# raywan-110/AdaQP

Hardware: NVIDIA H100
Metric: epochs_per_sec (higher is better)
Workload: dtype f32

## Files before the change

### adaqp_b200/_lib.py

```python
from __future__ import annotations

import ctypes as C
import os

import numpy as np

HERE = os.path.dirname(os.path.abspath(__file__))
LIB_PATH = os.path.join(HERE, "libadaqp_b200.so")

c_void_p = C.c_void_p
i64 = C.c_int64
i32 = C.c_int32
u64 = C.c_uint64
u32 = C.c_uint32

ADAQP_ABI_VERSION = 7
MAX_PARTS = 64
LP_HUB_DEGREE = 256
IPC_HANDLE_BYTES = 64
ST_OK, ST_FLAG_TIMEOUT, ST_ACK_TIMEOUT = 0, 1, 2

SEND_ITEM_DTYPE = np.dtype([
    ("src_row", np.int32, (4,)), ("send_pos", np.int32, (4,)), ("dst_off", np.int64),
    ("param_pos", np.int32), ("group", np.int32), ("rel_offset", np.uint32),
    ("chan", np.int16), ("bits", np.int8), ("nrows", np.int8), ("_pad", np.int32)],
    align=True)
RECV_ITEM_DTYPE = np.dtype([
    ("dst_row", np.int32, (4,)), ("src_off", np.int64), ("param_pos", np.int32),
    ("chan", np.int16), ("bits", np.int8), ("nrows", np.int8)], align=True)
FP_ITEM_DTYPE = np.dtype([("src_row", np.int32), ("chan", np.int32), ("dst_row", np.int64)],
                         align=True)
# ... 31 lines not shown
    "adaqp_ipc_close": (C.c_int, [c_void_p]),
    "adaqp_can_access_peer": (C.c_int, [C.c_int]),
    "adaqp_send_quant": (C.c_int, [c_void_p, i64, i32, c_void_p, i64, c_void_p, i32, c_void_p,
                                   u64, u64, u32, c_void_p, c_void_p, u64, c_void_p]),
    "adaqp_recv_quant": (C.c_int, [c_void_p, i64, i32, c_void_p, i64, c_void_p, i32, u32,
                                   c_void_p, c_void_p, u64, c_void_p]),
    "adaqp_send_fp32": (C.c_int, [c_void_p, i64, i32, c_void_p, i64, c_void_p, i32, i64, u32,
                                  c_void_p, c_void_p, u64, c_void_p]),
    "adaqp_wait_flags": (C.c_int, [c_void_p, i32, u32, c_void_p, u64, c_void_p]),
    "adaqp_post_acks": (C.c_int, [c_void_p, i32, u32, c_void_p]),
    "adaqp_spmm_csr_f32": (C.c_int, [c_void_p, c_void_p, c_void_p, i64, i64, c_void_p, i64,
                                     c_void_p, c_void_p, C.c_int, C.c_int, i64, i64, i32,
                                     c_void_p, i64, c_void_p]),
    "adaqp_spmm_csr_seg_f32": (C.c_int, [c_void_p, c_void_p, c_void_p, c_void_p, c_void_p, i64, i64, c_void_p,
                                         i64, c_void_p, c_void_p, C.c_int, C.c_int, C.c_int, i64, i64, i32,
                                         c_void_p, i64, c_void_p, c_void_p]),
    "adaqp_row_live_f32": (C.c_int, [c_void_p, i64, i64, i32, c_void_p, c_void_p]),
    "adaqp_appnp_prop_f32": (C.c_int, [c_void_p, c_void_p, c_void_p, c_void_p, c_void_p, i64, i64, c_void_p, i64,
                                       c_void_p, c_void_p, C.c_float, C.c_float, c_void_p, i64, c_void_p, i64, i32,
                                       C.c_int, i64, i64, i32, c_void_p, i64, c_void_p]),
    "adaqp_gemm_tf32x3_supported": (C.c_int, [i64, i32, i32, i64, i64, i64]),
    "adaqp_gemm_tf32x3_f32": (C.c_int, [c_void_p, i64, c_void_p, c_void_p, i64, c_void_p, i64, i32, i32, c_void_p, i64, c_void_p]),
    "adaqp_wgrad_tf32x3_supported": (C.c_int, [i64, i32, i32, i64, i64]),
    "adaqp_wgrad_tf32x3_grid": (C.c_int, [i64]),
    "adaqp_wgrad_tf32x3_f32": (C.c_int, [c_void_p, i64, c_void_p, i64, i64, i32, i32, c_void_p, i32, c_void_p]),
    "adaqp_ln_relu_grid": (C.c_int, [i64]),
    "adaqp_ln_relu_fwd_f32": (C.c_int, [c_void_p, i64, c_void_p, c_void_p, C.c_float, i64, i32, c_void_p, i64, c_void_p, c_void_p, c_void_p]),
    "adaqp_ln_relu_bwd_f32": (C.c_int, [c_void_p, i64, c_void_p, i64, c_void_p, c_void_p, c_void_p, c_void_p, i64, i32, c_void_p, i64,
                                        c_void_p, i32, c_void_p]),
    "adaqp_gather_rows_f32": (C.c_int, [c_void_p, i64, c_void_p, i64, i32, c_void_p, i64,
                                        c_void_p]),
# ... 103 lines not shown
```

### adaqp_b200/csrc/spmm.cu

```cuda
#include <cuda.h>

#include <mutex>
#include <unordered_map>

#include "common.cuh"

namespace {

constexpr int kWarps = 8;
constexpr int kThreads = kWarps * 32;
constexpr int kUnroll = 4;

constexpr int kHintStoreStreaming = 1;
constexpr int kHintIndexStreaming = 2;

template <int VEC> struct Vec;
template <> struct Vec<4> {
    static __device__ __forceinline__ void load(const float *p, float (&v)[4]) {
        const float4 t = __ldg(reinterpret_cast<const float4 *>(p)); v[0] = t.x; v[1] = t.y; v[2] = t.z; v[3] = t.w;
    }
    static __device__ __forceinline__ void store(float *p, const float (&v)[4]) {
        *reinterpret_cast<float4 *>(p) = make_float4(v[0], v[1], v[2], v[3]);
    }
    static __device__ __forceinline__ void store_cs(float *p, const float (&v)[4]) {
// ... 56 lines not shown
                        } else {                                                                                        \
_Pragma("unroll")                                                                                                       \
                            for (int e = 0; e < VEC; ++e) v[t][c][e] = 0.f;                                             \
                        }                                                                                               \
                    }                                                                                                   \
                }                                                                                                       \
_Pragma("unroll")                                                                                                       \
                for (int t = 0; t < UNROLL_; ++t)                                                                       \
_Pragma("unroll")                                                                                                       \
                    for (int c = 0; c < CHUNKS; ++c)                                                                    \
_Pragma("unroll")                                                                                                       \
                        for (int e = 0; e < VEC; ++e) acc[c][e] = __fmaf_rn(ww[t], v[t][c][e], acc[c][e]);              \
            }                                                                                                           \
        }

template <int VEC, int CHUNKS, bool SKIP>
__global__ void __launch_bounds__(kThreads)
spmm_csr_kernel(const int64_t *__restrict__ indptr, const int32_t *__restrict__ indices,
                const float *__restrict__ x0, int64_t ld0, int64_t n_split,
                const float *__restrict__ x1, int64_t ld1,
                const float *__restrict__ pre, const float *__restrict__ post,
                int mean, int add_self, int64_t row_begin, int64_t row_end, int F,
                float *__restrict__ out, int64_t ldo, unsigned long long *__restrict__ next_row, int rows_per_grab,
                const int64_t *__restrict__ seg_start, const int64_t *__restrict__ seg_end, int accumulate, int hints,
                const uint8_t *__restrict__ live) {
    const int lane = threadIdx.x & 31;
    bool colok[CHUNKS];
#pragma unroll
    for (int c = 0; c < CHUNKS; ++c) colok[c] = ((c * 32 + lane) * VEC) < F;

    const int64_t n_rows = row_end - row_begin;
    while (true) {
        unsigned long long grab = 0;
        if (lane == 0) grab = atomicAdd(next_row, (unsigned long long)rows_per_grab);
        grab = __shfl_sync(ADAQP_FULL_MASK, grab, 0);
        if ((int64_t)grab >= n_rows) break;
        const int64_t r_hi = ((int64_t)grab + rows_per_grab < n_rows) ? (int64_t)grab + rows_per_grab : n_rows;
    for (int64_t row = row_begin + (int64_t)grab; row < row_begin + r_hi; ++row) {
        float acc[CHUNKS][VEC];
#pragma unroll
        for (int c = 0; c < CHUNKS; ++c)
#pragma unroll
            for (int e = 0; e < VEC; ++e) acc[c][e] = 0.f;
        const int64_t row_b = __ldg(indptr + row), row_e = __ldg(indptr + row + 1);
        const int64_t b = seg_start ? __ldg(seg_start + row) : row_b;
        const int64_t e_ = seg_end ? __ldg(seg_end + row) : row_e;
        ADAQP_GATHER_SEGMENT(kUnroll, SKIP, live)
        if (add_self) {
            const float ws = pre ? __ldg(pre + row) : 1.f;
            const float *rp = (row < n_split) ? (x0 + row * ld0) : (x1 + (row - n_split) * ld1);
#pragma unroll
            for (int c = 0; c < CHUNKS; ++c) {
                if (colok[c]) {
// ... 96 lines not shown
            if (!colok[c]) continue;
            float r[VEC];
#pragma unroll
            for (int e = 0; e < VEC; ++e) {
                r[e] = __fmul_rn(acc[c][e], s);
                if (add_tele) r[e] = __fmaf_rn(alpha, addend[c][e], r[e]);
                else if (fold) r[e] = __fadd_rn(r[e], addend[c][e]);
                else if (accumulate) r[e] = __fadd_rn(addend[c][e], r[e]);
            }
            Vec<VEC>::store(orow + (c * 32 + lane) * VEC, r);
        }
    }
    frontier_release(next_row);
}

template <bool SKIP>
__global__ void __launch_bounds__(kThreads)
spmm_csr_sliced_kernel(const int64_t *__restrict__ indptr, const int32_t *__restrict__ indices,
                       const float *__restrict__ x0, int64_t ld0, int64_t n_split,
                       const float *__restrict__ x1, int64_t ld1,
                       const float *__restrict__ pre, const float *__restrict__ post,
                       int mean, int add_self, int64_t row_begin, int64_t row_end, int F, int slice_cols,
                       float *__restrict__ out, int64_t ldo, unsigned long long *__restrict__ next_row, int rows_per_grab,
                       const int64_t *__restrict__ seg_start, const int64_t *__restrict__ seg_end, int accumulate, int hints,
                       const uint8_t *__restrict__ live) {
    const int lane = threadIdx.x & 31;
    const int64_t n_rows = row_end - row_begin;
    const int64_t n_grabs = (n_rows + rows_per_grab - 1) / rows_per_grab;
    const int64_t n_units = n_grabs * ((F + slice_cols - 1) / slice_cols);
    while (true) {
        unsigned long long unit = 0;
        if (lane == 0) unit = atomicAdd(next_row, 1ull);
        unit = __shfl_sync(ADAQP_FULL_MASK, unit, 0);
        if ((int64_t)unit >= n_units) break;
        const int64_t slice = (int64_t)unit / n_grabs, grab = (int64_t)unit % n_grabs;
        const int col = (int)slice * slice_cols + lane * 4;
        const bool colok = lane * 4 < slice_cols && col < F;
        const int64_t r_lo = row_begin + grab * rows_per_grab;
        const int64_t r_hi = (r_lo + rows_per_grab < row_end) ? r_lo + rows_per_grab : row_end;
        for (int64_t row = r_lo; row < r_hi; ++row) {
            const int64_t row_b = __ldg(indptr + row), row_e = __ldg(indptr + row + 1);
            const int64_t b = seg_start ? __ldg(seg_start + row) : row_b;
            const int64_t e_ = seg_end ? __ldg(seg_end + row) : row_e;
            float acc[4] = {0.f, 0.f, 0.f, 0.f};
            for (int64_t j0 = b; j0 < e_; j0 += 32) {
                int n = (e_ - j0) < 32 ? (int)(e_ - j0) : 32;
                int u = 0;
                float w = 0.f;
                if (lane < n) {
                    u = (hints & kHintIndexStreaming) ? __ldcs(indices + j0 + lane) : __ldg(indices + j0 + lane);
                    w = pre ? __ldg(pre + u) : 1.f;
                }
                if constexpr (SKIP) n = compact_live_window(lane, n, n_split, live, u, w);
                for (int k = 0; k < n; k += kUnroll) {
                    float v[kUnroll][4];
// ... 557 lines not shown
    if (cudaMemset(p, 0, 2 * sizeof(unsigned long long)) != cudaSuccess) return nullptr;
    pairs.emplace(key, p);
    return p;
}

}

unsigned long long *adaqp_frontier_counter(int dev, cudaStream_t s) { return frontier_counter(dev, s); }

extern "C" {

int adaqp_spmm_csr_seg_f32(const int64_t *indptr, const int64_t *seg_start, const int64_t *seg_end,
                           const int32_t *indices, const float *x0, int64_t ld0,
                           int64_t n_split, const float *x1, int64_t ld1, const float *pre,
                           const float *post, int mean, int add_self, int accumulate, int64_t row_begin,
                           int64_t row_end, int32_t F, float *out, int64_t ldo, const uint8_t *live, void *stream) {
    ADAQP_REQUIRE(F > 0 && F <= 1024, ADAQP_ELIMIT, "adaqp_spmm_csr_f32: F=%d outside (0,1024]", F);
    ADAQP_REQUIRE(row_end >= row_begin && row_begin >= 0, ADAQP_EINVAL, "adaqp_spmm_csr_f32: bad row range");
    if (row_end == row_begin) return 0;
    ADAQP_REQUIRE(indptr && indices && x0 && out, ADAQP_EINVAL, "adaqp_spmm_csr_f32: null pointer");
    int vec = 4;
    auto fits = [&](int v) {
        if (F % v || ld0 % v || ldo % v) return false;
        if (!aligned(x0, v) || !aligned(out, v)) return false;
        if (x1 && (!aligned(x1, v) || (ld1 % v))) return false;
        return true;
    };
    while (vec > 1 && !fits(vec)) vec >>= 1;
    const int nchunks = (F + 32 * vec - 1) / (32 * vec);
    const int64_t rows = row_end - row_begin;
    const int sms = adaqp_sm_count() > 0 ? adaqp_sm_count() : 132;
    const AdaqpOptions &opt = adaqp_options();
    cudaStream_t s = (cudaStream_t)stream;
    const int impl = opt.spmm_impl;
    if (impl == 2 && vec == 4 && nchunks <= 8 && !seg_start && !seg_end && !accumulate) {
        auto launch = [&](auto kernel, int C) {
            const size_t smem = (size_t)kWarps * kStages * C * 512;
            int ctas_per_sm = (int)((200 * 1024) / (smem + 1024));
            if (ctas_per_sm > 4) ctas_per_sm = 4;
            if (ctas_per_sm < 1) ctas_per_sm = 1;
            int64_t g2 = (int64_t)sms * ctas_per_sm;
            const int64_t max_ctas = (rows + kWarps - 1) / kWarps;
            if (g2 > max_ctas) g2 = max_ctas;
            const int64_t chunk_nnz = 2048;
            cudaFuncSetAttribute(kernel, cudaFuncAttributeMaxDynamicSharedMemorySize, 200 * 1024);
            kernel<<<(unsigned)g2, kThreads, smem, s>>>(indptr, indices, x0, ld0, n_split, x1, ld1, pre, post, mean,
                                                        add_self, row_begin, row_end, F, out, ldo, chunk_nnz);
        };
        if (nchunks <= 1) launch(spmm_csr_ring_kernel<1>, 1);
        else if (nchunks <= 2) launch(spmm_csr_ring_kernel<2>, 2);
        else if (nchunks <= 3) launch(spmm_csr_ring_kernel<3>, 3);
        else if (nchunks <= 4) launch(spmm_csr_ring_kernel<4>, 4);
        else if (nchunks <= 6) launch(spmm_csr_ring_kernel<6>, 6);
        else launch(spmm_csr_ring_kernel<8>, 8);
        return adaqp_check_launch("spmm_csr_ring_kernel");
    }
    int dev = 0;
    ADAQP_CUDA(cudaGetDevice(&dev));
    unsigned long long *counter = frontier_counter(dev, s);
    ADAQP_REQUIRE(counter != nullptr, ADAQP_EINVAL, "adaqp_spmm_csr_seg_f32: row counter allocation failed");
    if ((impl == 3 || impl == 4) && vec == 4 && F <= 256 && nchunks <= 2) {
        CUtensorMap map0, map1;
        memset(&map0, 0, sizeof(map0));
        memset(&map1, 0, sizeof(map1));
        if (impl == 3) {
            const int64_t rows0 = n_split > 0 ? n_split : 1;
            int rc = make_row_map(&map0, x0, rows0, F, ld0);
            if (rc) return rc;
            if (x1) { rc = make_row_map(&map1, x1, (int64_t)1 << 31, F, ld1); if (rc) return rc; }
        }
        const uint32_t slot_bytes = 4u * ring_row_stride(F);
        int stages = (int)((200u * 1024u) / ((size_t)kRingWarps * (slot_bytes + sizeof(RingMeta) + 8)));
        if (stages > 8) stages = 8;
        ADAQP_REQUIRE(stages >= 2, ADAQP_ELIMIT, "adaqp_spmm_csr_seg_f32: ring does not fit shared memory");
        const size_t smem = (size_t)kRingWarps * stages * (slot_bytes + sizeof(RingMeta) + 8);
        int64_t grid = (rows + kRingWarps - 1) / kRingWarps;
        if (grid > sms) grid = sms;
        const int grab = opt.spmm_rows_per_grab > 0 ? opt.spmm_rows_per_grab : 4;
        auto launch = [&](auto kernel) {
            cudaFuncSetAttribute(kernel, cudaFuncAttributeMaxDynamicSharedMemorySize, (int)smem);
            kernel<<<(unsigned)grid, kRingThreads, smem, s>>>(map0, map1, indptr, indices, x0, ld0, n_split, x1, ld1, pre, post,
                                                             mean, add_self, row_begin, row_end, F, out, ldo, counter, grab,
                                                             seg_start, seg_end, accumulate, stages);
        };
        if (impl == 3) { if (nchunks <= 1) launch(spmm_csr_tma_kernel<1, true>); else launch(spmm_csr_tma_kernel<2, true>); }
        else { if (nchunks <= 1) launch(spmm_csr_tma_kernel<1, false>); else launch(spmm_csr_tma_kernel<2, false>); }
        return adaqp_check_launch("spmm_csr_tma_kernel");
    }
    const int64_t cta_cap = (int64_t)sms * (opt.spmm_ctas_per_sm > 0 ? opt.spmm_ctas_per_sm : 8);
    const int hints = opt.spmm_hints;
    int slice = 0;
    if (vec == 4) {
        slice = opt.spmm_slice_cols > 0 ? opt.spmm_slice_cols : auto_slice_cols(F);
        if (slice >= F) slice = 0;
        ADAQP_REQUIRE(slice == 0 || (slice % 4 == 0 && slice <= 128), ADAQP_EINVAL,
                      "adaqp_spmm_csr_seg_f32: slice width %d is not a multiple of 4 in [4, 128]", slice);
    }
    const int grab_rows = opt.spmm_rows_per_grab > 0 ? opt.spmm_rows_per_grab : 1;
    if (slice > 0) {
        const int grab = grab_rows;
        const int64_t units = ((rows + grab - 1) / grab) * ((F + slice - 1) / slice);
        int64_t grid = (units + kWarps - 1) / kWarps;
        if (grid > cta_cap) grid = cta_cap;
        auto launch_sliced = [&](auto kernel) {
            kernel<<<(unsigned)grid, kThreads, 0, s>>>(indptr, indices, x0, ld0, n_split, x1, ld1, pre, post, mean, add_self,
                                                       row_begin, row_end, F, slice, out, ldo, counter, grab, seg_start, seg_end,
                                                       accumulate, hints, live);
        };
        if (live) launch_sliced(spmm_csr_sliced_kernel<true>);
        else launch_sliced(spmm_csr_sliced_kernel<false>);
        return adaqp_check_launch("spmm_csr_sliced_kernel");
    }
    int64_t grid = (rows + kWarps - 1) / kWarps;
    const int grab_now = grab_rows;
    if (grid > cta_cap) grid = cta_cap;
#define CALL_SPMM(V, C)                                                                                                  \
    do {                                                                                                                 \
        if (live) spmm_csr_kernel<V, C, true><<<(unsigned)grid, kThreads, 0, s>>>(                                       \
            indptr, indices, x0, ld0, n_split, x1, ld1, pre, post, mean, add_self, row_begin, row_end, F, out, ldo,      \
            counter, grab_now, seg_start, seg_end, accumulate, hints, live);                                             \
        else spmm_csr_kernel<V, C, false><<<(unsigned)grid, kThreads, 0, s>>>(                                           \
            indptr, indices, x0, ld0, n_split, x1, ld1, pre, post, mean, add_self, row_begin, row_end, F, out, ldo,      \
            counter, grab_now, seg_start, seg_end, accumulate, hints, nullptr);                                          \
    } while (0)
    if (vec == 4) {
        if (nchunks <= 1) CALL_SPMM(4, 1);
        else if (nchunks <= 2) CALL_SPMM(4, 2);
        else if (nchunks <= 3) CALL_SPMM(4, 3);
        else if (nchunks <= 4) CALL_SPMM(4, 4);
        else if (nchunks <= 6) CALL_SPMM(4, 6);
        else CALL_SPMM(4, 8);
    } else if (vec == 2) {
        if (nchunks <= 2) CALL_SPMM(2, 2);
        else if (nchunks <= 4) CALL_SPMM(2, 4);
        else if (nchunks <= 6) CALL_SPMM(2, 6);
        else if (nchunks <= 10) CALL_SPMM(2, 10);
        else CALL_SPMM(2, 16);
    } else {
        if (nchunks <= 4) CALL_SPMM(1, 4);
        else if (nchunks <= 8) CALL_SPMM(1, 8);
        else if (nchunks <= 16) CALL_SPMM(1, 16);
        else CALL_SPMM(1, 32);
    }
#undef CALL_SPMM
    return adaqp_check_launch("spmm_csr_kernel");
}


int adaqp_spmm_csr_f32(const int64_t *indptr, const int32_t *indices, const float *x0, int64_t ld0,
                       int64_t n_split, const float *x1, int64_t ld1, const float *pre,
                       const float *post, int mean, int add_self, int64_t row_begin,
                       int64_t row_end, int32_t F, float *out, int64_t ldo, void *stream) {
    return adaqp_spmm_csr_seg_f32(indptr, nullptr, nullptr, indices, x0, ld0, n_split, x1, ld1, pre, post, mean,
                                  add_self, 0, row_begin, row_end, F, out, ldo, nullptr, stream);
}

int adaqp_row_live_f32(const float *x, int64_t ld, int64_t rows, int32_t F, uint8_t *live, void *stream) {
    ADAQP_REQUIRE(F > 0 && rows >= 0 && ld >= F, ADAQP_EINVAL, "adaqp_row_live_f32: bad shape rows=%lld F=%d ld=%lld",
                  (long long)rows, F, (long long)ld);
    if (rows == 0) return 0;
    ADAQP_REQUIRE(x && live, ADAQP_EINVAL, "adaqp_row_live_f32: null pointer");
    const int sms = adaqp_sm_count() > 0 ? adaqp_sm_count() : 132;
    int64_t grid = (rows + kWarps - 1) / kWarps;
    if (grid > (int64_t)sms * 8) grid = (int64_t)sms * 8;
    cudaStream_t s = (cudaStream_t)stream;
    if (F % 4 == 0 && ld % 4 == 0 && aligned(x, 4))
        row_live_kernel<4><<<(unsigned)grid, kThreads, 0, s>>>(x, ld, rows, F, live);
    else
        row_live_kernel<1><<<(unsigned)grid, kThreads, 0, s>>>(x, ld, rows, F, live);
// ... 92 lines not shown
```

### adaqp_b200/manager/graph.py

```python
from __future__ import annotations

from typing import Dict, Optional

import numpy as np
import torch

from .. import _lib


class LocalGraph(object):
    def __init__(self, indptr: np.ndarray, indices: np.ndarray, in_degrees: np.ndarray,
                 out_degrees: np.ndarray, n_inner: int, n_halo: int, device: torch.device):
        self.device = torch.device(device)
        self.n_inner, self.n_halo = int(n_inner), int(n_halo)
        self.indptr = torch.from_numpy(np.ascontiguousarray(indptr, np.int64)).to(self.device)
        self.indices = torch.from_numpy(np.ascontiguousarray(indices, np.int32)).to(self.device)
        self.nnz = int(self.indices.numel())
        ip = np.ascontiguousarray(indptr, np.int64)
        is_local = (np.asarray(indices) < self.n_inner)
        csum = np.concatenate([[0], np.cumsum(is_local, dtype=np.int64)])
        self.halo_split = torch.from_numpy(ip[:-1] + (csum[ip[1:]] - csum[ip[:-1]])).to(self.device)
        self.ndata: Dict[str, torch.Tensor] = {
            "in_degrees": torch.from_numpy(np.ascontiguousarray(in_degrees)).to(self.device),
            "out_degrees": torch.from_numpy(np.ascontiguousarray(out_degrees)).to(self.device),
# ... 4 lines not shown
            "in_-0.5": ind.pow(-0.5).contiguous(), "out_-0.5": outd.pow(-0.5).contiguous(),
            "out_-1": torch.pow(outd, -1).contiguous(), "in_+1_-1": torch.pow(ind + 1, -1).contiguous(),
            "out_+1_-1": torch.pow(outd + 1, -1).contiguous(),
        }

    def num_nodes(self) -> int:
        return self.n_inner + self.n_halo

    def num_edges(self) -> int:
        return self.nnz

    def to(self, device):
        return self if torch.device(device) == self.device else NotImplemented


def spmm(graph: LocalGraph, x_local: torch.Tensor, x_halo: Optional[torch.Tensor],
         pre: Optional[torch.Tensor], post: Optional[torch.Tensor], mean: bool = False,
         add_self: bool = False, row_begin: int = 0, row_end: Optional[int] = None,
         out: Optional[torch.Tensor] = None, stream=None, part: Optional[str] = None,
         live: Optional[torch.Tensor] = None) -> torch.Tensor:
    L = _lib.load()
    row_end = graph.n_inner if row_end is None else int(row_end)
    F = int(x_local.shape[1])
    assert x_local.dtype == torch.float32 and x_local.stride(1) == 1
    if out is None:
        out = torch.empty((row_end - row_begin, F), dtype=torch.float32, device=x_local.device)
    if x_halo is not None and x_halo.shape[0] == 0:
        x_halo = None
    seg_start = seg_end = None
    accumulate = 0
    if part == "local":
        seg_end = graph.halo_split.data_ptr()
    elif part == "halo":
        assert out is not None, "the halo part accumulates into the output of the local part"
        seg_start = graph.halo_split.data_ptr()
        accumulate, add_self = 1, False
    elif part is not None:
        raise ValueError(part)
    if live is not None:
        assert live.dtype == torch.uint8 and live.is_contiguous() and live.numel() >= graph.n_inner
    rc = L.adaqp_spmm_csr_seg_f32(
        graph.indptr.data_ptr(), seg_start, seg_end, graph.indices.data_ptr(), x_local.data_ptr(),
        x_local.stride(0), graph.n_inner, x_halo.data_ptr() if x_halo is not None else None,
        x_halo.stride(0) if x_halo is not None else 0,
        pre.data_ptr() if pre is not None else None, post.data_ptr() if post is not None else None,
        1 if mean else 0, 1 if add_self else 0, accumulate, int(row_begin), row_end, F, out.data_ptr(),
        out.stride(0), live.data_ptr() if live is not None else None, _lib.stream_ptr(stream))
    _lib.check(rc, "adaqp_spmm_csr_seg_f32")
    return out


def row_live(x: torch.Tensor, out: Optional[torch.Tensor] = None, stream=None) -> torch.Tensor:
    assert x.dtype == torch.float32 and x.dim() == 2 and x.stride(1) == 1
    rows, F = int(x.shape[0]), int(x.shape[1])
    if out is None:
        out = torch.empty(rows, dtype=torch.uint8, device=x.device)
    assert out.dtype == torch.uint8 and out.is_contiguous() and out.numel() >= rows
    if rows == 0:
        return out
    rc = _lib.load().adaqp_row_live_f32(x.data_ptr(), x.stride(0), rows, F, out.data_ptr(), _lib.stream_ptr(stream))
    _lib.check(rc, "adaqp_row_live_f32")
    return out
# ... 41 lines not shown
```

### adaqp_b200/model/ops.py

```python
from __future__ import annotations

from typing import Any, Tuple

import torch
from torch import Tensor
from torch.autograd import Function

from .. import gat, gatv2, sage_pool
from ..communicator import Communicator as comm
from ..communicator.p2p import attn_keys, pool_arg_key, push_key
from ..helper import BitType, ProprogationMode
from ..manager import DecompGraph
from ..manager import GraphEngine as engine
from ..manager.graph import ACC_FOLD, ACC_ON, ACC_READ, LocalGraph, appnp_prop, row_live, spmm
from ..manager.graphEngine import RowRange
from .op_util import halo_exchange, msg_all2all_GLOO


def _split(graph, feats: Tensor, x_halo: Tensor = None):
    g = graph.graph if isinstance(graph, RowRange) else graph
    if x_halo is None and feats.shape[0] > g.n_inner:
        return g, feats[:g.n_inner], feats[g.n_inner:]
    return g, feats, x_halo


def _run(g, x_local, x_halo, pre, post, mean, add_self, lo, hi, out=None, part=None, live=None):
    if isinstance(g, LocalGraph):
        return spmm(g, x_local, x_halo, pre, post, mean=mean, add_self=add_self, row_begin=lo, row_end=hi, out=out,
                    part=part, live=live)
    from ..manager.graph_cpu import spmm_cpu
    res = spmm_cpu(g, x_local, x_halo, pre, post, mean=mean, add_self=add_self, row_begin=lo, row_end=hi)
    if out is not None:
        out.copy_(res)
        return out
    return res


def GCN_aggregation(graph, feats: Tensor, mode: ProprogationMode = ProprogationMode.Forward,
                    x_halo: Tensor = None, out: Tensor = None, part: str = None, live: Tensor = None) -> Tensor:
    g, x_local, x_halo = _split(graph, feats, x_halo)
    lo, hi = (graph.begin, graph.end) if isinstance(graph, RowRange) else (0, g.n_inner)
    if mode == ProprogationMode.Forward:
        pre, post = g.norm["out_-0.5"], g.norm["in_-0.5"]
    elif mode == ProprogationMode.Backward:
        pre, post = g.norm["in_-0.5"], g.norm["out_-0.5"]
    else:
        raise ValueError(f"Invalid mode {mode}")
    return _run(g, x_local, x_halo, pre, post, False, False, lo, hi, out, part, live)


def SAGE_aggregation(graph, feats: Tensor, mode: ProprogationMode = ProprogationMode.Forward,
                     aggregator_type="mean", x_halo: Tensor = None, out: Tensor = None, part: str = None,
                     live: Tensor = None) -> Tensor:
    g, x_local, x_halo = _split(graph, feats, x_halo)
    lo, hi = (graph.begin, graph.end) if isinstance(graph, RowRange) else (0, g.n_inner)
    if mode == ProprogationMode.Forward:
        if aggregator_type == "mean":
            return _run(g, x_local, x_halo, None, None, True, False, lo, hi, out, part, live)
        if aggregator_type == "gcn":
            return _run(g, x_local, x_halo, None, g.norm["in_+1_-1"], False, True, lo, hi, out, part, live)
    elif mode == ProprogationMode.Backward:
        if aggregator_type == "mean":
            return _run(g, x_local, x_halo, g.norm["out_-1"], None, False, False, lo, hi, out, part, live)
        if aggregator_type == "gcn":
            return _run(g, x_local, x_halo, g.norm["out_+1_-1"], None, False, True, lo, hi, out, part, live)
    else:
        raise ValueError(f"Invalid mode {mode}")
    raise ValueError(f"Invalid aggregator_type {aggregator_type}")


def _aggregate(class_name: str, graph, x_local, x_halo, mode, out, part=None, live=None):
    if class_name == "DistAggConv":
        return GCN_aggregation(graph, x_local, mode=mode, x_halo=x_halo, out=out, part=part, live=live)
    if class_name == "DistAggSAGE":
        return SAGE_aggregation(graph, x_local, mode=mode, aggregator_type=engine.ctx.agg_type, x_halo=x_halo, out=out,
                                part=part, live=live)
    raise ValueError(f"Invalid class_name {class_name}")


def _eval_layer0(class_name: str, ctx, local_messages: Tensor, graph, layer: int, is_train: bool):
    import os
    from ..assigner import Assigner as assigner
    eng = engine.ctx
    fn = decomposed_graph_propagation if eng.use_parallel else full_graph_propagation
    usable = (not is_train and layer == 0 and os.environ.get("ADAQP_EVAL_CACHE", "1") != "0"
              and not (assigner.ctx is not None and assigner.ctx.is_tracing))
    if not usable:
        return fn(ctx, local_messages, graph, layer, is_train, ProprogationMode.Forward, class_name)
    if local_messages is not eng.feats:
        return fn(ctx, local_messages, graph, layer, is_train, ProprogationMode.Forward, class_name)
    key = (class_name, local_messages._version, tuple(local_messages.shape), id(graph),
# ... 50 lines not shown
def _skip_zero_rows() -> bool:
    global _SKIP
    if _SKIP is None:
        import os
        _SKIP = os.environ.get("ADAQP_SKIP_ZERO_ROWS", "1") != "0"
    return _SKIP


def _live_rows(local_messages: Tensor, layer: int, mode: ProprogationMode):
    top = getattr(engine.ctx, "top_layer", None)
    if mode != ProprogationMode.Backward or layer != top or not local_messages.is_cuda or not _skip_zero_rows():
        return None
    return row_live(local_messages)


def _finish(ctx, out: Tensor, layer: int, mode: ProprogationMode):
    if mode == ProprogationMode.Forward:
        ctx.saved = layer
        return out
    return out, None, None, None


def full_graph_propagation(ctx, local_messages: Tensor, graph, layer: int, is_train: bool,
                           mode: ProprogationMode, class_name: str):
    name = f"forward{layer}" if mode == ProprogationMode.Forward else f"backward{layer}"
    local_messages = local_messages.contiguous()
    timer = engine.ctx.timer
    g = graph.full if isinstance(graph, DecompGraph) else graph
    if comm.ctx.transport == "p2p":
        quant = engine.ctx.bit_type == BitType.QUANT and is_train
        with timer.record_events(f"{name}_quantization" if quant else f"{name}_communication"):
            pend = halo_exchange(local_messages, name, is_train)
        with timer.record_events(f"{name}_full_aggregation"):
            live = _live_rows(local_messages, layer, mode)
            out = _aggregate(class_name, g, local_messages, pend.halo, mode, None, live=live)
        pend.release()
    else:
        send_messages = local_messages[engine.ctx.total_send_idx]
        remote = msg_all2all_GLOO(send_messages, name, is_train)
        with timer.record(f"{name}_full_aggregation"):
            out = _aggregate(class_name, g, local_messages, remote, mode, None)
    return _finish(ctx, out, layer, mode)


def decomposed_graph_propagation(ctx, local_messages: Tensor, graph, layer: int, is_train: bool,
                                 mode: ProprogationMode, class_name: str):
    assert isinstance(graph, DecompGraph), f"graph must be a DecompGraph, but got {type(graph)}"
    name = f"forward{layer}" if mode == ProprogationMode.Forward else f"backward{layer}"
    local_messages = local_messages.contiguous()
    eng, timer = engine.ctx, engine.ctx.timer
# ... 5 lines not shown
        with timer.record(f"{name}_central_aggregation"):
            _aggregate(class_name, graph.central_graph, local_messages, None, mode, out[:eng.num_central])
        remote = response.get() if response is not None else msg_all2all_GLOO(send_messages, name, is_train)
        with timer.record(f"{name}_marginal_aggregation"):
            _aggregate(class_name, graph.marginal_graph, local_messages, remote, mode, out[eng.num_central:])
        return _finish(ctx, out, layer, mode)
    main, side = torch.cuda.current_stream(), eng.marginal_stream
    quant = eng.bit_type == BitType.QUANT and is_train
    ready = torch.cuda.Event()
    ready.record(main)
    side.wait_event(ready)
    with timer.record_events(f"{name}_quantization" if quant else f"{name}_communication", stream=side):
        pend = halo_exchange(local_messages, name, is_train, stream=side)
    landed = torch.cuda.Event(enable_timing=True)
    landed.record(side)
    out = local_messages.new_empty((eng.num_inner, local_messages.shape[1]))
    with timer.record_events(f"{name}_central_aggregation"):
        live = _live_rows(local_messages, layer, mode)
        _aggregate(class_name, graph.central_graph, local_messages, None, mode, out[:eng.num_central], live=live)
    if _split_marginal():
        with timer.record_events(f"{name}_marginal_aggregation_local"):
            _aggregate(class_name, graph.marginal_graph, local_messages, None, mode, out[eng.num_central:],
                       part="local", live=live)
        overlappable_done = torch.cuda.Event(enable_timing=True)
        overlappable_done.record(main)
        timer.record_exposed(name, overlappable_done, landed)
        main.wait_event(landed)
        with timer.record_events(f"{name}_marginal_aggregation_halo"):
            _aggregate(class_name, graph.marginal_graph, local_messages, pend.halo, mode, out[eng.num_central:],
                       part="halo", live=live)
    else:
        central_done = torch.cuda.Event(enable_timing=True)
        central_done.record(main)
        timer.record_exposed(name, central_done, landed)
        main.wait_event(landed)
        with timer.record_events(f"{name}_marginal_aggregation"):
            _aggregate(class_name, graph.marginal_graph, local_messages, pend.halo, mode, out[eng.num_central:],
                       live=live)
    pend.release()
    local_messages.record_stream(side)
    return _finish(ctx, out, layer, mode)


def _gat_exchange(rows: Tensor, name: str, is_train: bool, scalars: Tensor, aux_key: str, stream=None):
    ex = comm.ctx.comm_buffer.p2p
    ex.post_send_fp(aux_key, scalars, stream=stream)
    pend = halo_exchange(rows, name, is_train, stream=stream)
    return pend, ex.complete_recv_fp(aux_key, stream=stream)


def _gat_release(pend, aux_key: str):
    pend.release()
    if aux_key is not None:
# ... 304 lines not shown
```

### adaqp_b200/trainer/runtime_util.py

```python
from __future__ import annotations

import logging
import time
from typing import Any, List, Tuple, Union

import numpy as np
import torch
import torch.distributed as dist
from torch import Tensor, nn
from torch.optim import Optimizer

from ..assigner import Assigner as assigner
from ..communicator import Communicator as comm
from ..helper import BitType
from ..manager import GraphEngine as engine

_nccl_group = None


def setup_logger(log_file, level=logging.INFO, with_file=True):
    lg = logging.getLogger("trainer")
    lg.setLevel(level)
    if with_file and not any(isinstance(h, logging.FileHandler) for h in lg.handlers):
        fh = logging.FileHandler(log_file)
        fh.setFormatter(logging.Formatter("%(asctime)s %(levelname)s %(message)s"))
        lg.addHandler(fh)
    return lg


def fix_seed(seed: int = 0):
# ... 58 lines not shown
        buf.p2p.check_status()


def train_for_one_epoch(epoch: int, graph, model: nn.Module, input_data: Tensor, labels: Tensor,
                        optimizer: Optimizer, criterion: Union[nn.Module, Any], total_num_training_samples: int,
                        train_mask: Tensor) -> Tuple[Any, Tensor, List[float], float]:
    overhead = 0.0
    if epoch % assigner.ctx.assign_cycle == 1 and epoch != 1:
        if assigner.ctx.scheme in ["adaptive", "random"] and engine.ctx.bit_type == BitType.QUANT:
            logging.getLogger("trainer").info(f"<epoch {epoch}, updating bit-width...>")
            t0 = time.time()
            comm.ctx.update_buffer(assigner.ctx.get_assignment(engine.ctx.send_idx))
            overhead = time.time() - t0
    epoch_start = time.time()
    model.train()
    logits = model(graph, input_data)
    loss = criterion(logits[train_mask], labels[train_mask]) / total_num_training_samples
    optimizer.zero_grad()
    loss.backward()
    update_start = time.time()
    average_gradients(model)
    reduce_time = time.time() - update_start
    optimizer.step()
    if comm.ctx.device.type == "cuda":
        torch.cuda.synchronize()
    epoch_time = time.time() - epoch_start
    _check_exchange_status()
    engine.ctx.last_exposed_comm_ms = engine.ctx.timer.exposed_comm_ms()
    traced_time = engine.ctx.timer.epoch_traced_time()
    engine.ctx.timer.clear()
    traced_time.insert(0, epoch_time)
# ... 53 lines not shown
```

### include/adaqp_b200.h

```cpp
#ifndef ADAQP_B200_H
#define ADAQP_B200_H

#include <stddef.h>
#include <stdint.h>

#ifdef __cplusplus
extern "C" {
#endif

#define ADAQP_ABI_VERSION 7

#define ADAQP_EINVAL (-1)
#define ADAQP_EALIGN (-2)
#define ADAQP_ELIMIT (-3)

#define ADAQP_ST_OK 0u
#define ADAQP_ST_FLAG_TIMEOUT 1u
#define ADAQP_ST_ACK_TIMEOUT 2u

int adaqp_abi_version(void);
const char *adaqp_last_error(void);
int adaqp_sm_count(void);
int adaqp_set_option(const char *name, int64_t value);
int adaqp_get_option(const char *name, int64_t *value);

// ... 89 lines not shown
                     uint32_t *status, uint64_t timeout_ns, void *stream);
int adaqp_post_acks(uint32_t *const *acks, int32_t n, uint32_t seq, void *stream);

int adaqp_spmm_csr_f32(const int64_t *indptr, const int32_t *indices,
                       const float *x0, int64_t ld0, int64_t n_split,
                       const float *x1, int64_t ld1,
                       const float *pre, const float *post, int mean, int add_self,
                       int64_t row_begin, int64_t row_end, int32_t F,
                       float *out, int64_t ldo, void *stream);

int adaqp_spmm_csr_seg_f32(const int64_t *indptr, const int64_t *seg_start, const int64_t *seg_end,
                           const int32_t *indices, const float *x0, int64_t ld0, int64_t n_split,
                           const float *x1, int64_t ld1, const float *pre, const float *post,
                           int mean, int add_self, int accumulate, int64_t row_begin,
                           int64_t row_end, int32_t F, float *out, int64_t ldo, const uint8_t *live,
                           void *stream);

int adaqp_row_live_f32(const float *x, int64_t ld, int64_t rows, int32_t F, uint8_t *live, void *stream);

int adaqp_appnp_prop_f32(const int64_t *indptr, const int64_t *seg_start, const int64_t *seg_end,
                         const int32_t *indices, const float *x0, int64_t ld0, int64_t n_split, const float *x1,
                         int64_t ld1, const float *pre, const float *post, float scale, float alpha,
                         const float *tele, int64_t ldt, float *acc, int64_t lda, int32_t acc_mode, int accumulate,
                         int64_t row_begin, int64_t row_end, int32_t F, float *out, int64_t ldo, void *stream);

int adaqp_gemm_tf32x3_supported(int64_t M, int32_t N, int32_t K, int64_t lda, int64_t ldb, int64_t ldc);
int adaqp_gemm_tf32x3_f32(const float *A, int64_t lda, const float *Bt_hi, const float *Bt_lo, int64_t ldb,
                          const float *bias, int64_t M, int32_t N, int32_t K, float *C, int64_t ldc, void *stream);

int adaqp_wgrad_tf32x3_supported(int64_t M, int32_t N, int32_t K, int64_t ldy, int64_t ldx);
int adaqp_wgrad_tf32x3_grid(int64_t M);
// ... 72 lines not shown
```

Baseline: 7.410.

## Aggregate only training-loss rows in the top forward layer via row lists

Adds a row-list mode to the CSR SpMM kernels and, during training, limits top-layer forward aggregation to the rows selected by the train mask. The other output rows are zero-filled. This removes SpMM work for rows whose outputs never feed the loss. It adds a host-side mask-to-list conversion, which is cached by mask version, and a zeroing pass. It also assumes the top layer's other rows are unused, which holds only when the loss reads masked logits and the top layer is purely an aggregation.

```diff
diff --git a/adaqp_b200/_lib.py b/adaqp_b200/_lib.py
--- a/adaqp_b200/_lib.py
+++ b/adaqp_b200/_lib.py
@@ -14,7 +14,7 @@
 u64 = C.c_uint64
 u32 = C.c_uint32
 
-ADAQP_ABI_VERSION = 7
+ADAQP_ABI_VERSION = 8
 MAX_PARTS = 64
 LP_HUB_DEGREE = 256
 IPC_HANDLE_BYTES = 64
@@ -76,7 +76,7 @@
                                      c_void_p, i64, c_void_p]),
     "adaqp_spmm_csr_seg_f32": (C.c_int, [c_void_p, c_void_p, c_void_p, c_void_p, c_void_p, i64, i64, c_void_p,
                                          i64, c_void_p, c_void_p, C.c_int, C.c_int, C.c_int, i64, i64, i32,
-                                         c_void_p, i64, c_void_p, c_void_p]),
+                                         c_void_p, i64, c_void_p, c_void_p, i64, c_void_p]),
     "adaqp_row_live_f32": (C.c_int, [c_void_p, i64, i64, i32, c_void_p, c_void_p]),
     "adaqp_appnp_prop_f32": (C.c_int, [c_void_p, c_void_p, c_void_p, c_void_p, c_void_p, i64, i64, c_void_p, i64,
                                        c_void_p, c_void_p, C.c_float, C.c_float, c_void_p, i64, c_void_p, i64, i32,
diff --git a/adaqp_b200/csrc/spmm.cu b/adaqp_b200/csrc/spmm.cu
--- a/adaqp_b200/csrc/spmm.cu
+++ b/adaqp_b200/csrc/spmm.cu
@@ -94,7 +94,7 @@
             }                                                                                                           \
         }
 
-template <int VEC, int CHUNKS, bool SKIP>
+template <int VEC, int CHUNKS, bool SKIP, bool LIST>
 __global__ void __launch_bounds__(kThreads)
 spmm_csr_kernel(const int64_t *__restrict__ indptr, const int32_t *__restrict__ indices,
                 const float *__restrict__ x0, int64_t ld0, int64_t n_split,
@@ -103,20 +103,22 @@
                 int mean, int add_self, int64_t row_begin, int64_t row_end, int F,
                 float *__restrict__ out, int64_t ldo, unsigned long long *__restrict__ next_row, int rows_per_grab,
                 const int64_t *__restrict__ seg_start, const int64_t *__restrict__ seg_end, int accumulate, int hints,
-                const uint8_t *__restrict__ live) {
+                const uint8_t *__restrict__ live, const int32_t *__restrict__ rows, int64_t n_list) {
     const int lane = threadIdx.x & 31;
     bool colok[CHUNKS];
 #pragma unroll
     for (int c = 0; c < CHUNKS; ++c) colok[c] = ((c * 32 + lane) * VEC) < F;
 
-    const int64_t n_rows = row_end - row_begin;
+    const int64_t n_rows = LIST ? n_list : row_end - row_begin;
+    const int64_t pos_base = LIST ? 0 : row_begin;
     while (true) {
         unsigned long long grab = 0;
         if (lane == 0) grab = atomicAdd(next_row, (unsigned long long)rows_per_grab);
         grab = __shfl_sync(ADAQP_FULL_MASK, grab, 0);
         if ((int64_t)grab >= n_rows) break;
         const int64_t r_hi = ((int64_t)grab + rows_per_grab < n_rows) ? (int64_t)grab + rows_per_grab : n_rows;
-    for (int64_t row = row_begin + (int64_t)grab; row < row_begin + r_hi; ++row) {
+    for (int64_t pos = pos_base + (int64_t)grab; pos < pos_base + r_hi; ++pos) {
+        const int64_t row = LIST ? (int64_t)__ldg(rows + pos) : pos;
         float acc[CHUNKS][VEC];
 #pragma unroll
         for (int c = 0; c < CHUNKS; ++c)
@@ -243,7 +245,7 @@
     frontier_release(next_row);
 }
 
-template <bool SKIP>
+template <bool SKIP, bool LIST>
 __global__ void __launch_bounds__(kThreads)
 spmm_csr_sliced_kernel(const int64_t *__restrict__ indptr, const int32_t *__restrict__ indices,
                        const float *__restrict__ x0, int64_t ld0, int64_t n_split,
@@ -252,9 +254,10 @@
                        int mean, int add_self, int64_t row_begin, int64_t row_end, int F, int slice_cols,
                        float *__restrict__ out, int64_t ldo, unsigned long long *__restrict__ next_row, int rows_per_grab,
                        const int64_t *__restrict__ seg_start, const int64_t *__restrict__ seg_end, int accumulate, int hints,
-                       const uint8_t *__restrict__ live) {
+                       const uint8_t *__restrict__ live, const int32_t *__restrict__ rows, int64_t n_list) {
     const int lane = threadIdx.x & 31;
-    const int64_t n_rows = row_end - row_begin;
+    const int64_t n_rows = LIST ? n_list : row_end - row_begin;
+    const int64_t pos_begin = LIST ? 0 : row_begin, pos_end = LIST ? n_list : row_end;
     const int64_t n_grabs = (n_rows + rows_per_grab - 1) / rows_per_grab;
     const int64_t n_units = n_grabs * ((F + slice_cols - 1) / slice_cols);
     while (true) {
@@ -265,9 +268,10 @@
         const int64_t slice = (int64_t)unit / n_grabs, grab = (int64_t)unit % n_grabs;
         const int col = (int)slice * slice_cols + lane * 4;
         const bool colok = lane * 4 < slice_cols && col < F;
-        const int64_t r_lo = row_begin + grab * rows_per_grab;
-        const int64_t r_hi = (r_lo + rows_per_grab < row_end) ? r_lo + rows_per_grab : row_end;
-        for (int64_t row = r_lo; row < r_hi; ++row) {
+        const int64_t r_lo = pos_begin + grab * rows_per_grab;
+        const int64_t r_hi = (r_lo + rows_per_grab < pos_end) ? r_lo + rows_per_grab : pos_end;
+        for (int64_t pos = r_lo; pos < r_hi; ++pos) {
+            const int64_t row = LIST ? (int64_t)__ldg(rows + pos) : pos;
             const int64_t row_b = __ldg(indptr + row), row_e = __ldg(indptr + row + 1);
             const int64_t b = seg_start ? __ldg(seg_start + row) : row_b;
             const int64_t e_ = seg_end ? __ldg(seg_end + row) : row_e;
@@ -855,10 +859,16 @@
                            const int32_t *indices, const float *x0, int64_t ld0,
                            int64_t n_split, const float *x1, int64_t ld1, const float *pre,
                            const float *post, int mean, int add_self, int accumulate, int64_t row_begin,
-                           int64_t row_end, int32_t F, float *out, int64_t ldo, const uint8_t *live, void *stream) {
+                           int64_t row_end, int32_t F, float *out, int64_t ldo, const uint8_t *live,
+                           const int32_t *rows, int64_t n_list, void *stream) {
     ADAQP_REQUIRE(F > 0 && F <= 1024, ADAQP_ELIMIT, "adaqp_spmm_csr_f32: F=%d outside (0,1024]", F);
     ADAQP_REQUIRE(row_end >= row_begin && row_begin >= 0, ADAQP_EINVAL, "adaqp_spmm_csr_f32: bad row range");
+    ADAQP_REQUIRE(!rows || (n_list >= 0 && n_list <= row_end - row_begin), ADAQP_EINVAL,
+                  "adaqp_spmm_csr_seg_f32: row list of %lld ids for a range of %lld rows", (long long)n_list,
+                  (long long)(row_end - row_begin));
+    ADAQP_REQUIRE(!(rows && live), ADAQP_EINVAL, "adaqp_spmm_csr_seg_f32: a row list and row liveness together");
     if (row_end == row_begin) return 0;
+    if (rows && n_list == 0) return 0;
     ADAQP_REQUIRE(indptr && indices && x0 && out, ADAQP_EINVAL, "adaqp_spmm_csr_f32: null pointer");
     int vec = 4;
     auto fits = [&](int v) {
@@ -869,19 +879,19 @@
     };
     while (vec > 1 && !fits(vec)) vec >>= 1;
     const int nchunks = (F + 32 * vec - 1) / (32 * vec);
-    const int64_t rows = row_end - row_begin;
+    const int64_t n_rows = row_end - row_begin;
     const int sms = adaqp_sm_count() > 0 ? adaqp_sm_count() : 132;
     const AdaqpOptions &opt = adaqp_options();
     cudaStream_t s = (cudaStream_t)stream;
     const int impl = opt.spmm_impl;
-    if (impl == 2 && vec == 4 && nchunks <= 8 && !seg_start && !seg_end && !accumulate) {
+    if (impl == 2 && !rows && vec == 4 && nchunks <= 8 && !seg_start && !seg_end && !accumulate) {
         auto launch = [&](auto kernel, int C) {
             const size_t smem = (size_t)kWarps * kStages * C * 512;
             int ctas_per_sm = (int)((200 * 1024) / (smem + 1024));
             if (ctas_per_sm > 4) ctas_per_sm = 4;
             if (ctas_per_sm < 1) ctas_per_sm = 1;
             int64_t g2 = (int64_t)sms * ctas_per_sm;
-            const int64_t max_ctas = (rows + kWarps - 1) / kWarps;
+            const int64_t max_ctas = (n_rows + kWarps - 1) / kWarps;
             if (g2 > max_ctas) g2 = max_ctas;
             const int64_t chunk_nnz = 2048;
             cudaFuncSetAttribute(kernel, cudaFuncAttributeMaxDynamicSharedMemorySize, 200 * 1024);
@@ -900,7 +910,7 @@
     ADAQP_CUDA(cudaGetDevice(&dev));
     unsigned long long *counter = frontier_counter(dev, s);
     ADAQP_REQUIRE(counter != nullptr, ADAQP_EINVAL, "adaqp_spmm_csr_seg_f32: row counter allocation failed");
-    if ((impl == 3 || impl == 4) && vec == 4 && F <= 256 && nchunks <= 2) {
+    if ((impl == 3 || impl == 4) && !rows && vec == 4 && F <= 256 && nchunks <= 2) {
         CUtensorMap map0, map1;
         memset(&map0, 0, sizeof(map0));
         memset(&map1, 0, sizeof(map1));
@@ -915,7 +925,7 @@
         if (stages > 8) stages = 8;
         ADAQP_REQUIRE(stages >= 2, ADAQP_ELIMIT, "adaqp_spmm_csr_seg_f32: ring does not fit shared memory");
         const size_t smem = (size_t)kRingWarps * stages * (slot_bytes + sizeof(RingMeta) + 8);
-        int64_t grid = (rows + kRingWarps - 1) / kRingWarps;
+        int64_t grid = (n_rows + kRingWarps - 1) / kRingWarps;
         if (grid > sms) grid = sms;
         const int grab = opt.spmm_rows_per_grab > 0 ? opt.spmm_rows_per_grab : 4;
         auto launch = [&](auto kernel) {
@@ -938,31 +948,36 @@
                       "adaqp_spmm_csr_seg_f32: slice width %d is not a multiple of 4 in [4, 128]", slice);
     }
     const int grab_rows = opt.spmm_rows_per_grab > 0 ? opt.spmm_rows_per_grab : 1;
+    const int64_t work_rows = rows ? n_list : n_rows;
     if (slice > 0) {
         const int grab = grab_rows;
-        const int64_t units = ((rows + grab - 1) / grab) * ((F + slice - 1) / slice);
+        const int64_t units = ((work_rows + grab - 1) / grab) * ((F + slice - 1) / slice);
         int64_t grid = (units + kWarps - 1) / kWarps;
         if (grid > cta_cap) grid = cta_cap;
         auto launch_sliced = [&](auto kernel) {
             kernel<<<(unsigned)grid, kThreads, 0, s>>>(indptr, indices, x0, ld0, n_split, x1, ld1, pre, post, mean, add_self,
                                                        row_begin, row_end, F, slice, out, ldo, counter, grab, seg_start, seg_end,
-                                                       accumulate, hints, live);
+                                                       accumulate, hints, live, rows, n_list);
         };
-        if (live) launch_sliced(spmm_csr_sliced_kernel<true>);
-        else launch_sliced(spmm_csr_sliced_kernel<false>);
+        if (rows) launch_sliced(spmm_csr_sliced_kernel<false, true>);
+        else if (live) launch_sliced(spmm_csr_sliced_kernel<true, false>);
+        else launch_sliced(spmm_csr_sliced_kernel<false, false>);
         return adaqp_check_launch("spmm_csr_sliced_kernel");
     }
-    int64_t grid = (rows + kWarps - 1) / kWarps;
+    int64_t grid = (work_rows + kWarps - 1) / kWarps;
     const int grab_now = grab_rows;
     if (grid > cta_cap) grid = cta_cap;
 #define CALL_SPMM(V, C)                                                                                                  \
     do {                                                                                                                 \
-        if (live) spmm_csr_kernel<V, C, true><<<(unsigned)grid, kThreads, 0, s>>>(                                       \
+        if (rows) spmm_csr_kernel<V, C, false, true><<<(unsigned)grid, kThreads, 0, s>>>(                                \
             indptr, indices, x0, ld0, n_split, x1, ld1, pre, post, mean, add_self, row_begin, row_end, F, out, ldo,      \
-            counter, grab_now, seg_start, seg_end, accumulate, hints, live);                                             \
-        else spmm_csr_kernel<V, C, false><<<(unsigned)grid, kThreads, 0, s>>>(                                           \
+            counter, grab_now, seg_start, seg_end, accumulate, hints, nullptr, rows, n_list);                            \
+        else if (live) spmm_csr_kernel<V, C, true, false><<<(unsigned)grid, kThreads, 0, s>>>(                           \
             indptr, indices, x0, ld0, n_split, x1, ld1, pre, post, mean, add_self, row_begin, row_end, F, out, ldo,      \
-            counter, grab_now, seg_start, seg_end, accumulate, hints, nullptr);                                          \
+            counter, grab_now, seg_start, seg_end, accumulate, hints, live, nullptr, 0);                                 \
+        else spmm_csr_kernel<V, C, false, false><<<(unsigned)grid, kThreads, 0, s>>>(                                    \
+            indptr, indices, x0, ld0, n_split, x1, ld1, pre, post, mean, add_self, row_begin, row_end, F, out, ldo,      \
+            counter, grab_now, seg_start, seg_end, accumulate, hints, nullptr, nullptr, 0);                              \
     } while (0)
     if (vec == 4) {
         if (nchunks <= 1) CALL_SPMM(4, 1);
@@ -993,7 +1008,7 @@
                        const float *post, int mean, int add_self, int64_t row_begin,
                        int64_t row_end, int32_t F, float *out, int64_t ldo, void *stream) {
     return adaqp_spmm_csr_seg_f32(indptr, nullptr, nullptr, indices, x0, ld0, n_split, x1, ld1, pre, post, mean,
-                                  add_self, 0, row_begin, row_end, F, out, ldo, nullptr, stream);
+                                  add_self, 0, row_begin, row_end, F, out, ldo, nullptr, nullptr, 0, stream);
 }
 
 int adaqp_row_live_f32(const float *x, int64_t ld, int64_t rows, int32_t F, uint8_t *live, void *stream) {
diff --git a/adaqp_b200/manager/graph.py b/adaqp_b200/manager/graph.py
--- a/adaqp_b200/manager/graph.py
+++ b/adaqp_b200/manager/graph.py
@@ -42,17 +42,65 @@
         return self if torch.device(device) == self.device else NotImplemented
 
 
+class RowList(object):
+
+    def __init__(self, ids: torch.Tensor, host: np.ndarray):
+        assert ids.dtype == torch.int32 and ids.dim() == 1 and ids.is_contiguous() and ids.numel() == host.size
+        self.ids, self._host = ids, host
+        self.n = int(host.size)
+        self.first = int(host[0]) if self.n else None
+        self.last = int(host[-1]) if self.n else None
+
+    def _cut(self, k: int) -> int:
+        return int(np.searchsorted(self._host, k, side="left"))
+
+    def below(self, n: int) -> "RowList":
+        k = self._cut(n)
+        return RowList(self.ids[:k], self._host[:k])
+
+    def from_(self, n: int) -> "RowList":
+        k = self._cut(n)
+        return RowList(self.ids[k:], self._host[k:])
+
+    def __len__(self) -> int:
+        return self.n
+
+
+def row_list(mask: torch.Tensor, n_rows: int, device) -> RowList:
+    m = mask.detach().cpu()
+    if m.dtype == torch.bool:
+        if m.dim() != 1 or m.numel() != n_rows:
+            raise ValueError(f"bool row mask of shape {tuple(m.shape)} for {n_rows} rows")
+        host = torch.nonzero(m).flatten().numpy().astype(np.int64)
+    else:
+        if m.is_floating_point() or m.is_complex():
+            raise ValueError(f"row mask of dtype {m.dtype}: a bool mask or integer row ids")
+        host = np.unique(m.flatten().to(torch.int64).numpy())
+    if host.size and (host[0] < 0 or host[-1] >= n_rows):
+        raise ValueError(f"row ids [{int(host[0])}, {int(host[-1])}] outside [0, {n_rows})")
+    host = host.astype(np.int32)
+    return RowList(torch.from_numpy(host).to(device), host)
+
+
 def spmm(graph: LocalGraph, x_local: torch.Tensor, x_halo: Optional[torch.Tensor],
          pre: Optional[torch.Tensor], post: Optional[torch.Tensor], mean: bool = False,
          add_self: bool = False, row_begin: int = 0, row_end: Optional[int] = None,
          out: Optional[torch.Tensor] = None, stream=None, part: Optional[str] = None,
-         live: Optional[torch.Tensor] = None) -> torch.Tensor:
+         live: Optional[torch.Tensor] = None, rows: Optional[RowList] = None) -> torch.Tensor:
     L = _lib.load()
     row_end = graph.n_inner if row_end is None else int(row_end)
     F = int(x_local.shape[1])
     assert x_local.dtype == torch.float32 and x_local.stride(1) == 1
     if out is None:
         out = torch.empty((row_end - row_begin, F), dtype=torch.float32, device=x_local.device)
+    n_list = 0
+    if rows is not None:
+        assert live is None, "a row list and row liveness are not combined"
+        assert rows.ids.dtype == torch.int32 and rows.ids.is_contiguous() and rows.ids.device == x_local.device
+        if rows.n == 0:
+            return out
+        assert row_begin <= rows.first and rows.last < row_end, (rows.first, rows.last, row_begin, row_end)
+        n_list = rows.n
     if x_halo is not None and x_halo.shape[0] == 0:
         x_halo = None
     seg_start = seg_end = None
@@ -73,7 +121,8 @@
         x_halo.stride(0) if x_halo is not None else 0,
         pre.data_ptr() if pre is not None else None, post.data_ptr() if post is not None else None,
         1 if mean else 0, 1 if add_self else 0, accumulate, int(row_begin), row_end, F, out.data_ptr(),
-        out.stride(0), live.data_ptr() if live is not None else None, _lib.stream_ptr(stream))
+        out.stride(0), live.data_ptr() if live is not None else None,
+        rows.ids.data_ptr() if rows is not None else None, n_list, _lib.stream_ptr(stream))
     _lib.check(rc, "adaqp_spmm_csr_seg_f32")
     return out
 
diff --git a/adaqp_b200/model/ops.py b/adaqp_b200/model/ops.py
--- a/adaqp_b200/model/ops.py
+++ b/adaqp_b200/model/ops.py
@@ -1,6 +1,7 @@
 from __future__ import annotations
 
-from typing import Any, Tuple
+import contextlib
+from typing import Any, Optional, Tuple
 
 import torch
 from torch import Tensor
@@ -12,7 +13,7 @@
 from ..helper import BitType, ProprogationMode
 from ..manager import DecompGraph
 from ..manager import GraphEngine as engine
-from ..manager.graph import ACC_FOLD, ACC_ON, ACC_READ, LocalGraph, appnp_prop, row_live, spmm
+from ..manager.graph import ACC_FOLD, ACC_ON, ACC_READ, LocalGraph, RowList, appnp_prop, row_list, row_live, spmm
 from ..manager.graphEngine import RowRange
 from .op_util import halo_exchange, msg_all2all_GLOO
 
@@ -24,10 +25,11 @@
     return g, feats, x_halo
 
 
-def _run(g, x_local, x_halo, pre, post, mean, add_self, lo, hi, out=None, part=None, live=None):
+def _run(g, x_local, x_halo, pre, post, mean, add_self, lo, hi, out=None, part=None, live=None, rows=None):
     if isinstance(g, LocalGraph):
         return spmm(g, x_local, x_halo, pre, post, mean=mean, add_self=add_self, row_begin=lo, row_end=hi, out=out,
-                    part=part, live=live)
+                    part=part, live=live, rows=rows)
+    assert rows is None, "row lists are a device-path feature"
     from ..manager.graph_cpu import spmm_cpu
     res = spmm_cpu(g, x_local, x_halo, pre, post, mean=mean, add_self=add_self, row_begin=lo, row_end=hi)
     if out is not None:
@@ -37,7 +39,8 @@
 
 
 def GCN_aggregation(graph, feats: Tensor, mode: ProprogationMode = ProprogationMode.Forward,
-                    x_halo: Tensor = None, out: Tensor = None, part: str = None, live: Tensor = None) -> Tensor:
+                    x_halo: Tensor = None, out: Tensor = None, part: str = None, live: Tensor = None,
+                    rows: RowList = None) -> Tensor:
     g, x_local, x_halo = _split(graph, feats, x_halo)
     lo, hi = (graph.begin, graph.end) if isinstance(graph, RowRange) else (0, g.n_inner)
     if mode == ProprogationMode.Forward:
@@ -46,35 +49,35 @@
         pre, post = g.norm["in_-0.5"], g.norm["out_-0.5"]
     else:
         raise ValueError(f"Invalid mode {mode}")
-    return _run(g, x_local, x_halo, pre, post, False, False, lo, hi, out, part, live)
+    return _run(g, x_local, x_halo, pre, post, False, False, lo, hi, out, part, live, rows)
 
 
 def SAGE_aggregation(graph, feats: Tensor, mode: ProprogationMode = ProprogationMode.Forward,
                      aggregator_type="mean", x_halo: Tensor = None, out: Tensor = None, part: str = None,
-                     live: Tensor = None) -> Tensor:
+                     live: Tensor = None, rows: RowList = None) -> Tensor:
     g, x_local, x_halo = _split(graph, feats, x_halo)
     lo, hi = (graph.begin, graph.end) if isinstance(graph, RowRange) else (0, g.n_inner)
     if mode == ProprogationMode.Forward:
         if aggregator_type == "mean":
-            return _run(g, x_local, x_halo, None, None, True, False, lo, hi, out, part, live)
+            return _run(g, x_local, x_halo, None, None, True, False, lo, hi, out, part, live, rows)
         if aggregator_type == "gcn":
-            return _run(g, x_local, x_halo, None, g.norm["in_+1_-1"], False, True, lo, hi, out, part, live)
+            return _run(g, x_local, x_halo, None, g.norm["in_+1_-1"], False, True, lo, hi, out, part, live, rows)
     elif mode == ProprogationMode.Backward:
         if aggregator_type == "mean":
-            return _run(g, x_local, x_halo, g.norm["out_-1"], None, False, False, lo, hi, out, part, live)
+            return _run(g, x_local, x_halo, g.norm["out_-1"], None, False, False, lo, hi, out, part, live, rows)
         if aggregator_type == "gcn":
-            return _run(g, x_local, x_halo, g.norm["out_+1_-1"], None, False, True, lo, hi, out, part, live)
+            return _run(g, x_local, x_halo, g.norm["out_+1_-1"], None, False, True, lo, hi, out, part, live, rows)
     else:
         raise ValueError(f"Invalid mode {mode}")
     raise ValueError(f"Invalid aggregator_type {aggregator_type}")
 
 
-def _aggregate(class_name: str, graph, x_local, x_halo, mode, out, part=None, live=None):
+def _aggregate(class_name: str, graph, x_local, x_halo, mode, out, part=None, live=None, rows=None):
     if class_name == "DistAggConv":
-        return GCN_aggregation(graph, x_local, mode=mode, x_halo=x_halo, out=out, part=part, live=live)
+        return GCN_aggregation(graph, x_local, mode=mode, x_halo=x_halo, out=out, part=part, live=live, rows=rows)
     if class_name == "DistAggSAGE":
         return SAGE_aggregation(graph, x_local, mode=mode, aggregator_type=engine.ctx.agg_type, x_halo=x_halo, out=out,
-                                part=part, live=live)
+                                part=part, live=live, rows=rows)
     raise ValueError(f"Invalid class_name {class_name}")
 
 
@@ -155,6 +158,36 @@
     return row_live(local_messages)
 
 
+_LOSS_MASK: Optional[Tensor] = None
+
+
+@contextlib.contextmanager
+def loss_rows(mask: Tensor):
+    global _LOSS_MASK
+    prev = _LOSS_MASK
+    _LOSS_MASK = mask
+    try:
+        yield
+    finally:
+        _LOSS_MASK = prev
+
+
+def _loss_row_list(local_messages: Tensor, layer: int, is_train: bool,
+                   mode: ProprogationMode) -> Optional[Tuple[RowList, Optional[RowList], Optional[RowList]]]:
+    mask, eng = _LOSS_MASK, engine.ctx
+    if (mask is None or not is_train or mode != ProprogationMode.Forward or layer != getattr(eng, "top_layer", None)
+            or not local_messages.is_cuda or comm.ctx.transport != "p2p"):
+        return None
+    key = (mask._version, eng.num_inner, eng.num_central if eng.use_parallel else None, local_messages.device)
+    cache = getattr(eng, "_loss_rows_cache", None)
+    if cache is None or cache[0] is not mask or cache[1] != key:
+        rows = row_list(mask, eng.num_inner, local_messages.device)
+        split = eng.num_central if eng.use_parallel else None
+        views = (rows, rows.below(split), rows.from_(split)) if split is not None else (rows, None, None)
+        eng._loss_rows_cache = cache = (mask, key, views)
+    return cache[2]
+
+
 def _finish(ctx, out: Tensor, layer: int, mode: ProprogationMode):
     if mode == ProprogationMode.Forward:
         ctx.saved = layer
@@ -173,8 +206,14 @@
         with timer.record_events(f"{name}_quantization" if quant else f"{name}_communication"):
             pend = halo_exchange(local_messages, name, is_train)
         with timer.record_events(f"{name}_full_aggregation"):
-            live = _live_rows(local_messages, layer, mode)
-            out = _aggregate(class_name, g, local_messages, pend.halo, mode, None, live=live)
+            listed = _loss_row_list(local_messages, layer, is_train, mode)
+            if listed is not None:
+                out = local_messages.new_zeros((g.n_inner, local_messages.shape[1]))
+                if listed[0].n:
+                    _aggregate(class_name, g, local_messages, pend.halo, mode, out, rows=listed[0])
+            else:
+                live = _live_rows(local_messages, layer, mode)
+                out = _aggregate(class_name, g, local_messages, pend.halo, mode, None, live=live)
         pend.release()
     else:
         send_messages = local_messages[engine.ctx.total_send_idx]
@@ -210,29 +249,41 @@
         pend = halo_exchange(local_messages, name, is_train, stream=side)
     landed = torch.cuda.Event(enable_timing=True)
     landed.record(side)
-    out = local_messages.new_empty((eng.num_inner, local_messages.shape[1]))
+    listed = _loss_row_list(local_messages, layer, is_train, mode)
+    _, central_rows, marginal_rows = listed if listed is not None else (None, None, None)
+    run_central = listed is None or central_rows.n > 0
+    run_marginal = listed is None or marginal_rows.n > 0
+    if listed is None:
+        out = local_messages.new_empty((eng.num_inner, local_messages.shape[1]))
     with timer.record_events(f"{name}_central_aggregation"):
+        if listed is not None:
+            out = local_messages.new_zeros((eng.num_inner, local_messages.shape[1]))
         live = _live_rows(local_messages, layer, mode)
-        _aggregate(class_name, graph.central_graph, local_messages, None, mode, out[:eng.num_central], live=live)
+        if run_central:
+            _aggregate(class_name, graph.central_graph, local_messages, None, mode, out[:eng.num_central], live=live,
+                       rows=central_rows)
     if _split_marginal():
         with timer.record_events(f"{name}_marginal_aggregation_local"):
-            _aggregate(class_name, graph.marginal_graph, local_messages, None, mode, out[eng.num_central:],
-                       part="local", live=live)
+            if run_marginal:
+                _aggregate(class_name, graph.marginal_graph, local_messages, None, mode, out[eng.num_central:],
+                           part="local", live=live, rows=marginal_rows)
         overlappable_done = torch.cuda.Event(enable_timing=True)
         overlappable_done.record(main)
         timer.record_exposed(name, overlappable_done, landed)
         main.wait_event(landed)
         with timer.record_events(f"{name}_marginal_aggregation_halo"):
-            _aggregate(class_name, graph.marginal_graph, local_messages, pend.halo, mode, out[eng.num_central:],
-                       part="halo", live=live)
+            if run_marginal:
+                _aggregate(class_name, graph.marginal_graph, local_messages, pend.halo, mode, out[eng.num_central:],
+                           part="halo", live=live, rows=marginal_rows)
     else:
         central_done = torch.cuda.Event(enable_timing=True)
         central_done.record(main)
         timer.record_exposed(name, central_done, landed)
         main.wait_event(landed)
         with timer.record_events(f"{name}_marginal_aggregation"):
-            _aggregate(class_name, graph.marginal_graph, local_messages, pend.halo, mode, out[eng.num_central:],
-                       live=live)
+            if run_marginal:
+                _aggregate(class_name, graph.marginal_graph, local_messages, pend.halo, mode, out[eng.num_central:],
+                           live=live, rows=marginal_rows)
     pend.release()
     local_messages.record_stream(side)
     return _finish(ctx, out, layer, mode)
diff --git a/adaqp_b200/trainer/runtime_util.py b/adaqp_b200/trainer/runtime_util.py
--- a/adaqp_b200/trainer/runtime_util.py
+++ b/adaqp_b200/trainer/runtime_util.py
@@ -14,6 +14,7 @@
 from ..communicator import Communicator as comm
 from ..helper import BitType
 from ..manager import GraphEngine as engine
+from ..model import ops
 
 _nccl_group = None
 
@@ -102,7 +103,8 @@
             overhead = time.time() - t0
     epoch_start = time.time()
     model.train()
-    logits = model(graph, input_data)
+    with ops.loss_rows(train_mask):
+        logits = model(graph, input_data)
     loss = criterion(logits[train_mask], labels[train_mask]) / total_num_training_samples
     optimizer.zero_grad()
     loss.backward()
diff --git a/include/adaqp_b200.h b/include/adaqp_b200.h
--- a/include/adaqp_b200.h
+++ b/include/adaqp_b200.h
@@ -8,7 +8,7 @@
 extern "C" {
 #endif
 
-#define ADAQP_ABI_VERSION 7
+#define ADAQP_ABI_VERSION 8
 
 #define ADAQP_EINVAL (-1)
 #define ADAQP_EALIGN (-2)
@@ -128,7 +128,7 @@
                            const float *x1, int64_t ld1, const float *pre, const float *post,
                            int mean, int add_self, int accumulate, int64_t row_begin,
                            int64_t row_end, int32_t F, float *out, int64_t ldo, const uint8_t *live,
-                           void *stream);
+                           const int32_t *rows, int64_t n_list, void *stream);
 
 int adaqp_row_live_f32(const float *x, int64_t ld, int64_t rows, int32_t F, uint8_t *live, void *stream);
 
```

Result: faster. 8.644, median of 6 (+16.7%).
